# paulffm/Continuous-Time-Diffusion-Models-for-Discrete-Data

Measured on AMD Instinct MI355X. Metric: tau-leaping sample-steps/s, higher is better.
Workload: dtype bf16; 1 GPU; MNIST tauLDR U-Net TauL step (config_tauUnet_mnist: D=784, S=256, 1000-step grid); batch_per_gpu=256, global_batch=256, D=784, S=256, parallelism=sample-sharded x1, no collective in the loop

## Files before the change

continuous-time-diffusion-models-for-discrete-data_amd/csrc/row_tile.hpp:

```cpp
#pragma once
#include <type_traits>

#include "common.hpp"

namespace ctdd {

using bf16x8 = __attribute__((ext_vector_type(8))) __bf16;
using bf16x2v = __attribute__((ext_vector_type(2))) __bf16;
using f32x2v = __attribute__((ext_vector_type(2))) float;
using f32x4 = __attribute__((ext_vector_type(4))) float;
using u32x4 = __attribute__((ext_vector_type(4))) unsigned;

constexpr int RT_UNIT = 9 * 512;

__device__ inline unsigned rt_pack2(float a, float b) {
  f32x2v v = {a, b};
  return __builtin_bit_cast(unsigned, __builtin_convertvector(v, bf16x2v));
}
__device__ inline int rt_again(int v) {
  asm volatile("" : "+v"(v));
  return v;
}

__device__ __attribute__((always_inline)) inline void rt_wload9(u32x4 (&dst)[3][3], const unsigned short* __restrict__ wrow, int u) {
// ... 30 lines not shown
    for (int y = 0; y < NPT; ++y) {
      if (FULL || y < H) {
        fload(fn[y + 2], o, y + 2);
#pragma unroll
        for (int dy = 0; dy < 3; ++dy)
#pragma unroll
          for (int t = 0; t < 3; ++t)
            acc[t][y] = __builtin_amdgcn_mfma_f32_16x16x32_bf16(__builtin_bit_cast(bf16x8, slot[dy][t]), fc[y + dy], acc[t][y], 0, 0, 0);
        __builtin_amdgcn_sched_barrier(0);
      }
    }
    if (!GUARD || u + 2 < nunits) rt_wload9(slot, wrow, u + 2);
    __builtin_amdgcn_sched_barrier(0);
  };
  bf16x8 F[2][NPT + 2];
  {
    const int o = xaddr();
#pragma unroll
    for (int r = 0; r < NPT + 2; ++r)
      if (FULL || r < H + 2) fload(F[0][r], o, r);
  }
  __builtin_amdgcn_s_waitcnt(0x0F70);
  int u0 = 0;
  for (; u0 + 4 <= nunits; u0 += 2) {
    step(wr[0], F[0], F[1], u0, std::false_type{});
    step(wr[1], F[1], F[0], u0 + 1, std::false_type{});
  }
  for (; u0 < nunits; u0 += 2) {
    step(wr[0], F[0], F[1], u0, std::true_type{});
    step(wr[1], F[1], F[0], u0 + 1, std::true_type{});
  }
}

}
```

continuous-time-diffusion-models-for-discrete-data_amd/csrc/unet_rows_kernels.hip:

```cpp
#include "row_tile.hpp"
#include "../../include/ctdd_unet.h"

namespace ctdd {
namespace {

constexpr int CR_THREADS = 256, CR_N = 96, CR_BAND = 14, CR_PITCH = 32, CR_RS = 224, CR_MAXW = 28, CR_MAXC = 384, CR_PIECE = 96;
constexpr int CR_SLAB = ((CR_BAND + 2) * CR_PITCH + 2) * CR_RS;
constexpr int CR_SCALE = CR_SLAB;
constexpr int CR_RED = CR_SCALE + 2 * CR_MAXC * 4;
constexpr int CR_TOTAL = CR_RED + 2 * CR_N * 2 * 8;
constexpr int CR_FB = 12;
static_assert(CR_BAND * CR_MAXW * CR_RS <= CR_SLAB, "the output image reuses the slab");

__device__ __attribute__((always_inline)) inline void cr_fill(unsigned char* sm, const unsigned short* __restrict__ src, int cs, int pc, int coff,
                                                             int y0, int H, int W) {
  const int t = threadIdx.x, noct = pc >> 3, npl = CR_THREADS / noct;
  if (t >= noct * npl) return;
  const int oct = t % noct, pl = t / noct;
  const float* scale = (const float*)(sm + CR_SCALE) + coff + oct * 8;
  const float* shift = scale + CR_MAXC;
  const float4 sc0 = *(const float4*)scale, sc1 = *(const float4*)(scale + 4);
  const float4 sh0 = *(const float4*)shift, sh1 = *(const float4*)(shift + 4);
  const f32x2v scv[4] = {{sc0.x, sc0.y}, {sc0.z, sc0.w}, {sc1.x, sc1.y}, {sc1.z, sc1.w}};
  const f32x2v shv[4] = {{sh0.x, sh0.y}, {sh0.z, sh0.w}, {sh1.x, sh1.y}, {sh1.z, sh1.w}};
  const int rlo = y0 == 0 ? 1 : 0, rhi = H - y0 < CR_BAND + 1 ? H - y0 : CR_BAND + 1;
  const unsigned npix = (unsigned)((rhi - rlo + 1) * W), uW = (unsigned)W;
  const unsigned short* sp = src + (size_t)((y0 - 1 + rlo) * W) * cs + oct * 8;
  unsigned char* dst = sm + (1 + rlo * CR_PITCH + 1) * CR_RS + oct * 16;
  for (unsigned p0 = (unsigned)pl; p0 < npix; p0 += (unsigned)(CR_FB * npl)) {
    u32x4 u[CR_FB];
#pragma unroll
    for (int k = 0; k < CR_FB; ++k) {
      const unsigned p = p0 + (unsigned)(k * npl);
      u[k] = *(const u32x4*)(sp + (size_t)(p < npix ? p : npix - 1) * cs);
    }
#pragma unroll
    for (int k = 0; k < CR_FB; ++k) {
      const unsigned p = p0 + (unsigned)(k * npl);
      unsigned ow[4];
#pragma unroll
      for (int j = 0; j < 4; ++j) {
        const f32x2v x = {__uint_as_float(u[k][j] << 16), __uint_as_float(u[k][j] & 0xFFFF0000u)};
        f32x2v y = __builtin_elementwise_fma(x, scv[j], shv[j]);
        const f32x2v z = y * (f32x2v){-1.4426950408889634f, -1.4426950408889634f};
        const f32x2v d = (f32x2v){__builtin_amdgcn_exp2f(z.x), __builtin_amdgcn_exp2f(z.y)} + (f32x2v){1.0f, 1.0f};
        y = y * (f32x2v){__builtin_amdgcn_rcpf(d.x), __builtin_amdgcn_rcpf(d.y)};
        ow[j] = rt_pack2(y.x, y.y);
      }
      const unsigned rr = p / uW, x = p - rr * uW;
      if (p < npix) *(uint4*)(dst + (rr * CR_PITCH + x) * CR_RS) = make_uint4(ow[0], ow[1], ow[2], ow[3]);
    }
  }
}

__device__ __attribute__((always_inline)) inline void cr_gemm_skip(f32x4 (&acc)[3][CR_BAND], u32x4 (&ws)[2][3], const unsigned short* __restrict__ wrow, int nsk,
                                                                  const unsigned short* __restrict__ r1, const unsigned short* __restrict__ r2,
                                                                  int C1, int C2, int xc, int lq, int y0, int H, int W) {
  const int nc1 = C1 >> 5;
  auto gload = [&](bf16x8 (&g)[CR_BAND], int u) {
    const int ue = u < nsk ? u : nsk - 1;
    const bool two = ue >= nc1;
    const unsigned char* base = (const unsigned char*)(two ? r2 : r1);
    const int cs = two ? C2 : C1, cb = (ue - (two ? nc1 : 0)) * 32 + lq * 8;
#pragma unroll
    for (int y = 0; y < CR_BAND; ++y) {
      const int ye = y0 + y < H ? y0 + y : H - 1;
      g[y] = *(const bf16x8*)(base + (unsigned)(((ye * W + xc) * cs + cb) * 2));
    }
  };
  auto step = [&](u32x4 (&slot)[3], bf16x8 (&gc)[CR_BAND], bf16x8 (&gn)[CR_BAND], int u, auto guard) {
    constexpr bool GUARD = decltype(guard)::value;
    if (GUARD && u >= nsk) return;
    gload(gn, u + 1);
#pragma unroll
    for (int y = 0; y < CR_BAND; ++y)
#pragma unroll
      for (int t = 0; t < 3; ++t)
        acc[t][y] = __builtin_amdgcn_mfma_f32_16x16x32_bf16(__builtin_bit_cast(bf16x8, slot[t]), gc[y], acc[t][y], 0, 0, 0);
    if (!GUARD || u + 2 < nsk) rt_wload3(slot, wrow, u + 2);
    __builtin_amdgcn_sched_barrier(0);
  };
  bf16x8 G[2][CR_BAND];
  gload(G[0], 0);
  __builtin_amdgcn_s_waitcnt(0x0F70);
  int u0 = 0;
  for (; u0 + 4 <= nsk; u0 += 2) {
    step(ws[0], G[0], G[1], u0, std::false_type{});
    step(ws[1], G[1], G[0], u0 + 1, std::false_type{});
  }
  for (; u0 < nsk; u0 += 2) {
    step(ws[0], G[0], G[1], u0, std::true_type{});
    step(ws[1], G[1], G[0], u0 + 1, std::true_type{});
  }
}

#ifdef CTDD_ROWS_STAMPS
#define CR_STAMP(i_)                                                                                      \
  do {                                                                                                    \
    unsigned long long t_;                                                                                \
    asm volatile("s_memtime %0\n\ts_waitcnt lgkmcnt(0)" : "=s"(t_)::"memory");                            \
    if (threadIdx.x == 0) ((unsigned long long*)a.out_stats)[(size_t)blockIdx.x * 8 + (i_)] = t_;         \
  } while (0)
#else
#define CR_STAMP(i_)
#endif

template <bool SKIP>
__global__ __launch_bounds__(CR_THREADS, 1) void k_conv_rows(const ctdd_conv_rows_args a) {
  extern __shared__ __attribute__((aligned(16))) unsigned char sm[];
  const int t = threadIdx.x;
  const int H = a.H, W = a.W, HW = H * W, C1 = a.C1, C2 = a.C2, C = C1 + C2;
  const int nbands = (H + CR_BAND - 1) / CR_BAND;
  const int b = blockIdx.x / nbands, y0 = (blockIdx.x - b * nbands) * CR_BAND;
  const int lane = t & 63, wv = t >> 6, lj = lane & 15, lq = lane >> 4, cg = wv >> 1, hh = wv & 1;
  const int nu3 = 3 * (C >> 5), nsk = SKIP ? (a.RC1 + a.RC2) >> 5 : 0;
  const unsigned short* wrow = (const unsigned short*)a.w + (size_t)cg * ((size_t)nu3 * RT_UNIT + (size_t)nsk * 1536) + lane * 8;
  u32x4 wr[2][3][3];
  CR_STAMP(0);

  rt_wload9(wr[0], wrow, 0);
  rt_wload9(wr[1], wrow, 1);
  for (int v = t; v < (CR_SLAB >> 4); v += CR_THREADS) *(uint4*)(sm + v * 16) = make_uint4(0, 0, 0, 0);
  {
    float* scale = (float*)(sm + CR_SCALE);
    float* shift = scale + CR_MAXC;
    const int cgp = C / a.G;
    for (int c = t; c < C; c += CR_THREADS) {
      const int g0 = (c / cgp) * cgp;
      double s = 0.0, q = 0.0;
      for (int j = g0; j < g0 + cgp; ++j) {
        const double* st = j < C1 ? a.st1 + ((size_t)b * C1 + j) * 2 : a.st2 + ((size_t)b * C2 + (j - C1)) * 2;
        s += st[0]; q += st[1];
      }
      const double n = (double)cgp * (double)HW;
      const double mean = s / n;
      const double var = fmax(q / n - mean * mean, 0.0);
      const float rstd = (float)(1.0 / sqrt(var + (double)a.eps));
      scale[c] = rstd * a.gamma[c];
      shift[c] = a.beta[c] - (float)mean * rstd * a.gamma[c];
    }
  }
  __syncthreads();
  CR_STAMP(1);

  const int fb = (1 + 16 * hh + lj) * CR_RS + lq * 16;
  f32x4 acc[3][CR_BAND];
#pragma unroll
  for (int tt = 0; tt < 3; ++tt)
#pragma unroll
    for (int y = 0; y < CR_BAND; ++y) acc[tt][y] = (f32x4){0.0f, 0.0f, 0.0f, 0.0f};

  int ub = 0;
  for (int s = 0; s < (C2 ? 2 : 1); ++s) {
    const int cs = s ? C2 : C1, coff = s ? C1 : 0;
    const unsigned short* src = (const unsigned short*)(s ? a.s2_bf16 : a.s1_bf16) + (size_t)b * HW * cs;
    for (int c0 = 0; c0 < cs; c0 += CR_PIECE) {
      const int pc = cs - c0 < CR_PIECE ? cs - c0 : CR_PIECE, nun = 3 * (pc >> 5);
      cr_fill(sm, src + c0, cs, pc, coff + c0, y0, H, W);
      __syncthreads();
      rt_gemm_rows<true, CR_RS, CR_PITCH>(acc, wr, wrow + (size_t)ub * RT_UNIT, nun, sm, fb, CR_BAND);
      __syncthreads();
      ub += nun;
      if (ub < nu3) {
        rt_wload9(wr[0], wrow + (size_t)ub * RT_UNIT, 0);
        rt_wload9(wr[1], wrow + (size_t)ub * RT_UNIT, 1);
      }
    }
  }
  CR_STAMP(2);

  if constexpr (SKIP) {
    const unsigned short* wsk = wrow + (size_t)nu3 * RT_UNIT;
    u32x4 ws[2][3];
    rt_wload3(ws[0], wsk, 0);
    if (nsk > 1) rt_wload3(ws[1], wsk, 1);
    const int cs_ = 16 * hh + rt_again(lj), xc = cs_ < 1 ? 0 : (cs_ > W ? W - 1 : cs_ - 1);
    cr_gemm_skip(acc, ws, wsk, nsk, (const unsigned short*)a.r1_bf16 + (size_t)b * HW * a.RC1,
                 (const unsigned short*)a.r2_bf16 + (size_t)b * HW * a.RC2, a.RC1, a.RC2, xc, lq, y0, H, W);
  }
  CR_STAMP(3);

  const int col = 16 * hh + rt_again(lj);
  const bool own = col >= 1 && col <= W;
  const int x2 = own ? col - 1 : 0;
  const int nrows = H - y0 < CR_BAND ? H - y0 : CR_BAND;
  double* red = (double*)(sm + CR_RED);
  uint2 rr[3][CR_BAND] = {};
  const bool res = !SKIP && a.res_bf16;
  if (res) {
    const unsigned short* rp = (const unsigned short*)a.res_bf16 + (size_t)b * HW * CR_N + cg * 48 + lq * 4;
#pragma unroll
    for (int y = 0; y < CR_BAND; ++y) {
      const unsigned short* rpy = rp + (size_t)(((y < nrows ? y0 + y : H - 1)) * W + x2) * CR_N;
#pragma unroll
      for (int tt = 0; tt < 3; ++tt) rr[tt][y] = *(const uint2*)(rpy + tt * 16);
    }
  }
#pragma unroll
  for (int tt = 0; tt < 3; ++tt) {
    const int n = cg * 48 + tt * 16 + lq * 4;
    const float4 bv = *(const float4*)(a.bias + n);
    const float4 tb = a.tbias ? *(const float4*)(a.tbias + (size_t)b * a.tb_stride + n) : make_float4(0.0f, 0.0f, 0.0f, 0.0f);
    const float add[4] = {bv.x + tb.x, bv.y + tb.y, bv.z + tb.z, bv.w + tb.w};
    const uint2 (&r)[CR_BAND] = rr[tt];
    float s[4] = {0.0f, 0.0f, 0.0f, 0.0f}, q[4] = {0.0f, 0.0f, 0.0f, 0.0f};
#pragma unroll
    for (int y = 0; y < CR_BAND; ++y) {
      if (y < nrows && own) {
        const f32x4 v = acc[tt][y];
        float o[4] = {v[0] + add[0], v[1] + add[1], v[2] + add[2], v[3] + add[3]};
        if (res) {
          o[0] += __uint_as_float(r[y].x << 16); o[1] += __uint_as_float(r[y].x & 0xFFFF0000u);
          o[2] += __uint_as_float(r[y].y << 16); o[3] += __uint_as_float(r[y].y & 0xFFFF0000u);
        }
#pragma unroll
        for (int i = 0; i < 4; ++i) { s[i] += o[i]; q[i] = fmaf(o[i], o[i], q[i]); }
        *(uint2*)(sm + (y * W + x2) * CR_RS + n * 2) = make_uint2(rt_pack2(o[0], o[1]), rt_pack2(o[2], o[3]));
      }
    }
#ifndef CTDD_ROWS_STAMPS
    if (a.out_stats) {
#pragma unroll
      for (int i = 0; i < 4; ++i) {
        double ds = (double)s[i], dq = (double)q[i];
#pragma unroll
        for (int m = 1; m < 16; m <<= 1) { ds += __shfl_xor(ds, m, WAVE); dq += __shfl_xor(dq, m, WAVE); }
        if (lj == 0) { red[(hh * CR_N + n + i) * 2] = ds; red[(hh * CR_N + n + i) * 2 + 1] = dq; }
      }
    }
#endif
  }
  __syncthreads();
  CR_STAMP(4);
  {
    constexpr int npc = CR_N / 8;
    unsigned short* out = (unsigned short*)a.out_bf16 + ((size_t)b * HW + (size_t)y0 * W) * CR_N;
    for (int v = t; v < nrows * W * npc; v += CR_THREADS) {
      const int p = v / npc, c0 = (v - p * npc) * 8;
      *(uint4*)(out + (size_t)p * CR_N + c0) = *(const uint4*)(sm + p * CR_RS + c0 * 2);
    }
#ifndef CTDD_ROWS_STAMPS
    if (a.out_stats && t < 2 * CR_N) atomicAdd(a.out_stats + (size_t)b * CR_N * 2 + t, red[t] + red[2 * CR_N + t]);
#endif
  }
  CR_STAMP(5);
}

}
}

using namespace ctdd;

extern "C" int ctdd_unet_conv_rows(const void* args_, int f32, void* stream) {
  CTDD_REQUIRE(args_, CTDD_EINVAL, "ctdd_unet_conv_rows: null arguments");
  const ctdd_conv_rows_args& a = *(const ctdd_conv_rows_args*)args_;
  CTDD_REQUIRE(f32 == 0, CTDD_ERANGE, "ctdd_unet_conv_rows: bf16 inference only (the fp32 mode keeps GroupNorm and convolution apart)");
  CTDD_REQUIRE(a.B > 0 && a.H > 0 && a.W >= 1 && a.W <= CR_MAXW, CTDD_ERANGE,
               "ctdd_unet_conv_rows: a grid of %dx%d pixels does not fit the row tiles (1 <= W <= 28)", a.H, a.W);
  const int nbands = (a.H + CR_BAND - 1) / CR_BAND;
  CTDD_REQUIRE((int64_t)a.B * nbands < ((int64_t)1 << 31) && (int64_t)a.H * a.W * CR_MAXC < ((int64_t)1 << 30), CTDD_ERANGE,
               "ctdd_unet_conv_rows: B=%d, %dx%d is over the 32-bit index range of the kernel", a.B, a.H, a.W);
  const int C = a.C1 + a.C2;
  CTDD_REQUIRE(a.N == CR_N && a.C1 > 0 && a.C1 % 32 == 0 && a.C2 >= 0 && a.C2 % 32 == 0 && C <= CR_MAXC && a.RC1 >= 0 && a.RC1 % 32 == 0 &&
                   a.RC2 >= 0 && a.RC2 % 32 == 0 && (a.RC2 == 0 || a.RC1 > 0) && a.RC1 + a.RC2 <= CR_MAXC, CTDD_ERANGE,
               "ctdd_unet_conv_rows: channel counts off the tile (N=%d, C1=%d, C2=%d, RC1=%d, RC2=%d; N = 96, sources in multiples of 32, <= 384 in all)",
               a.N, a.C1, a.C2, a.RC1, a.RC2);
  CTDD_REQUIRE(a.G > 0 && C % a.G == 0, CTDD_EINVAL, "ctdd_unet_conv_rows: %d groups do not divide %d channels", a.G, C);
  CTDD_REQUIRE(a.s1_bf16 && (a.C2 == 0 || a.s2_bf16) && (a.RC1 == 0 || a.r1_bf16) && (a.RC2 == 0 || a.r2_bf16) && a.gamma && a.beta && a.w &&
                   a.bias && a.out_bf16, CTDD_EINVAL, "ctdd_unet_conv_rows: null pointer");
  CTDD_REQUIRE(a.st1 && (a.C2 == 0 || a.st2), CTDD_EINVAL, "ctdd_unet_conv_rows: a GroupNorm source without statistics");
  auto al16 = [](const void* p) { return ((uintptr_t)p & 15) == 0; };
  CTDD_REQUIRE(al16(a.s1_bf16) && al16(a.s2_bf16) && al16(a.r1_bf16) && al16(a.r2_bf16) && al16(a.res_bf16) && al16(a.w) && al16(a.out_bf16) &&
                   al16(a.bias) && al16(a.tbias) && a.tb_stride % 4 == 0, CTDD_EINVAL, "ctdd_unet_conv_rows: tensors must be 16-byte aligned");
  CTDD_REQUIRE(!(a.RC1 > 0 && a.res_bf16), CTDD_EINVAL, "ctdd_unet_conv_rows: 1x1 segments and a residual in one call");
  static bool attr_done[2][16] = {};
  if (a.RC1 > 0) {
    ensure_lds_ceiling((const void*)k_conv_rows<true>, attr_done[1]);
    hipLaunchKernelGGL(k_conv_rows<true>, dim3(a.B * nbands), dim3(CR_THREADS), (size_t)CR_TOTAL, (hipStream_t)stream, a);
  } else {
    ensure_lds_ceiling((const void*)k_conv_rows<false>, attr_done[0]);
    hipLaunchKernelGGL(k_conv_rows<false>, dim3(a.B * nbands), dim3(CR_THREADS), (size_t)CR_TOTAL, (hipStream_t)stream, a);
  }
  return finish_launch("k_conv_rows");
}
```

continuous-time-diffusion-models-for-discrete-data_amd/ctdd/native.py:

```python
import ctypes as C
import os

import torch

_HERE = os.path.dirname(os.path.dirname(os.path.abspath(__file__)))
_LIB = None

BRANCH_CTELBO, BRANCH_CRM = 0, 1
LOGIT_TYPES = {"direct": 0, "reverse_prob": 1, "reverse_logscale": 2}
STEP_ORDINAL, STEP_CORRECTOR, STEP_COUNT_RAW, STEP_CRM, STEP_COUNT_JUMPS, STEP_BF16, STEP_LOGITS_BF16 = 1, 2, 4, 8, 16, 32, 64


class CtddError(RuntimeError):
    pass


def lib_path():
    return os.environ.get("CTDD_LIBRARY") or os.path.join(_HERE, "libctdd.so")


_P, _I, _F, _U64, _U32, _I64 = C.c_void_p, C.c_int, C.c_float, C.c_uint64, C.c_uint32, C.c_int64
_SIGS = {
    "ctdd_abi_version": ([], _I),
    "ctdd_last_error": ([], C.c_char_p),
# ... 25 lines not shown
    "ctdd_s256_step_table_bytes": ([], _I64),
    "ctdd_s256_prepare": ([_P, _P, _F, _I, _P, _P, _P, _P], _I),
    "ctdd_s256_prepare_crm": ([_P, _P, _I, _P, _P, _P, _P], _I),
    "ctdd_tauleap_step_s256": ([_P, _P, _P, _P, _P, _P, _F, _F, _U32, _U64, _U64, _I, _I, _P, _P, _P, _P], _I),
    "ctdd_tauleap_step_s256_rows": ([_P, _P, _P, _P, _P, _P, _F, _F, _U32, _U64, _U64, _I, _I, _P, _I, _P, _P, _P, _P], _I),
    "ctdd_crm_loss": ([_P, _P, _P, _P, _I, _I, _I, _I, _F, _F, _P, _P, _P, _P], _I),
    "ctdd_ctelbo_scratch_bytes": ([_I, _I, _I], _I64),
    "ctdd_ctelbo_loss": ([_P, _P, _P, _P, _P, _P, _I, _I, _I, _F, _F, _F, _P, _P, _P, _P], _I),
    "ctdd_ctelbo_loss_terms": ([_P, _P, _P, _P, _P, _P, _I, _I, _I, _F, _F, _F, _F, _P, _P, _P, _P], _I),
    "ctdd_ctelbo_loss_window": ([_P, _P, _P, _P, _P, _P, _I, _I, _I, _I, _I, _F, _F, _F, _F, _P, _P, _P, _P], _I),
    "ctdd_ctelbo_loss_masked": ([_P, _P, _P, _P, _P, _P, _P, _I, _I, _I, _F, _F, _F, _F, _P, _P, _P, _P], _I),
    "ctdd_score_elbo_loss": ([_P, _P, _P, _P, _P, _P, _I, _I, _I, _F, _F, _P, _P, _P, _P], _I),
    "ctdd_crm_loss_ll": ([_P, _P, _P, _I, _I, _I, _I, _F, _P, _P, _P, _P], _I),
    "ctdd_score_elbo_loss_ll": ([_P, _P, _P, _P, _P, _P, _I, _I, _I, _F, _F, _P, _P, _P, _P], _I),
    "ctdd_logprob_bwd": ([_I, _P, _P, _P, _P, _P, _F, _I, _I, _I, _P, _P, _P, _P], _I),
    "ctdd_crm_loss_masked": ([_P, _P, _P, _P, _P, _I, _I, _I, _I, _F, _F, _P, _P, _P, _P], _I),
    "ctdd_crm_loss_ll_masked": ([_P, _P, _P, _P, _I, _I, _I, _I, _F, _P, _P, _P, _P], _I),
    "ctdd_score_elbo_loss_masked": ([_P, _P, _P, _P, _P, _P, _P, _I, _I, _I, _F, _F, _P, _P, _P, _P], _I),
    "ctdd_score_elbo_loss_ll_masked": ([_P, _P, _P, _P, _P, _P, _P, _I, _I, _I, _F, _F, _P, _P, _P, _P], _I),
    "ctdd_opt_chunk_elems": ([], _I),
    "ctdd_adam_ema_step": ([_P, _P, _I, _F, _F, _F, _F, _I64, _F, _F, _P, _P], _I),
    "ctdd_grad_sumsq": ([_P, _P, _I, _P, _I, _P], _I),
    "ctdd_adam_ema_apply": ([_P, _P, _I, _F, _F, _F, _F, _I64, _F, _F, _P, _P], _I),
    "ctdd_d3pm_scratch_bytes": ([_I, _I, _I], _I64),
    "ctdd_d3pm_loss": ([_P, _P, _P, _P, _P, _P, _P, _I, _I, _I, _F, _F, _F, _P, _P, _P, _P, _P, _P], _I),
    "ctdd_d3pm_step": ([_P, _P, _P, _P, _P, _I, _I, _I, _I, _F, _P, _U64, _U64, _P, _P, _P, _P], _I),
    "ctdd_absorb_noise": ([_P, _P, _I, _I, _I, _U64, _U64, _P, _P], _I),
    "ctdd_absorb_scratch_bytes": ([], _I64),
    "ctdd_absorb_elbo_loss": ([_P, _P, _P, _P, _F, _I, _I, _I, _I, _P, _P, _P, _P], _I),
    "ctdd_absorb_step": ([_P, _P, _I, _I, _I, _I, _F, _U32, _U64, _U64, _P, _P, _P], _I),
}
UNET_EXPORTS = ("ctdd_unet_conv", "ctdd_unet_conv_patch", "ctdd_unet_conv_res", "ctdd_unet_conv_ring", "ctdd_unet_conv_up_phases", "ctdd_unet_upsample2x", "ctdd_unet_first_conv", "ctdd_unet_gn_apply", "ctdd_unet_gn_onepass", "ctdd_unet_channel_stats",
                "ctdd_unet_time", "ctdd_unet_time_uniform", "ctdd_unet_attention", "ctdd_unet_logistic_head", "ctdd_unet_resblock_small",
                "ctdd_unet_resblock_mid", "ctdd_unet_conv_rows", "ctdd_unet_conv_rows_head", "ctdd_unet_attention_block")
HOLLOW_EXPORTS = ("ctdd_gemm_bf16", "ctdd_hollow_small_linear", "ctdd_hollow_embed", "ctdd_hollow_layernorm", "ctdd_hollow_add", "ctdd_hollow_put_rows", "ctdd_hollow_attention", "ctdd_hollow_attention_bf16")
UNET_TRAIN_EXPORTS = ("ctdd_unet_wgrad", "ctdd_unet_gn_bwd", "ctdd_unet_dropout", "ctdd_unet_colsum", "ctdd_unet_sum_batch", "ctdd_unet_sum_jobs", "ctdd_unet_accumulate",
                      "ctdd_unet_downsum2x", "ctdd_unet_upsample2x_f32", "ctdd_unet_cast_rows", "ctdd_unet_attention_bwd",
                      "ctdd_unet_first_conv_wgrad", "ctdd_unet_first_conv_wgrad_scratch", "ctdd_unet_pack_weights",
                      "ctdd_unet_unpack_grads")
HOLLOW_TRAIN_EXPORTS = ("ctdd_hollow_layernorm_bwd", "ctdd_hollow_attention_train", "ctdd_hollow_attention_bwd", "ctdd_hollow_attention_train_bf16", "ctdd_hollow_attention_bwd_bf16", "ctdd_hollow_act", "ctdd_hollow_relu_bf16", "ctdd_hollow_colsum", "ctdd_hollow_dropout",
                        "ctdd_hollow_embed_bwd")
BERT_EXPORTS = ("ctdd_bert_embed", "ctdd_bert_gather", "ctdd_bert_attention_short",
                "ctdd_bert_embed_bwd", "ctdd_bert_gather_bwd",
                "ctdd_bert_embed_enum_bwd", "ctdd_bert_gather_enum_bwd",
                "ctdd_bert_attention_short_train", "ctdd_bert_attention_short_bwd")
EXPORTS = tuple(_SIGS) + UNET_EXPORTS + HOLLOW_EXPORTS + UNET_TRAIN_EXPORTS + HOLLOW_TRAIN_EXPORTS + BERT_EXPORTS


def load():
    global _LIB
    if _LIB is None:
        path = lib_path()
        if not os.path.exists(path):
            raise CtddError(f"{path} not found: build it with `python __graft_entry__.py` "
                            "(hipcc --offload-arch=gfx950); there is no CPU fallback")
        lib = C.CDLL(path)
        for name, (argt, rest) in _SIGS.items():
            fn = getattr(lib, name)
            fn.argtypes, fn.restype = argt, rest
        _LIB = lib
    return _LIB


def _ptr(t, dtype=None, name="tensor"):
    if t is None:
        return None
    if not isinstance(t, torch.Tensor):
# ... 639 lines not shown
```

continuous-time-diffusion-models-for-discrete-data_amd/ctdd/unet_engine.py:

```python
import contextlib
import ctypes as C

import torch

from . import native
from .plan_launch import bound_launch, graph_capture, ptr

_P, _I, _F = C.c_void_p, C.c_int, C.c_float
SEG_3x3, SEG_1x1, SEG_3x3_S2, SEG_3x3_UP = 0, 1, 2, 3


class _Seg(C.Structure):
    _fields_ = [("hi", _P), ("f32", _P), ("C", _I), ("kind", _I)]


class _ConvArgs(C.Structure):
    _fields_ = [("seg", _Seg * 3), ("nseg", _I), ("w_hi", _P), ("w_f32", _P), ("B", _I), ("H", _I), ("W", _I),
                ("Hin", _I), ("Win", _I), ("N", _I), ("Ktot", _I), ("bias", _P), ("tbias", _P), ("tb_stride", _I),
                ("res_f32", _P), ("res_bf16", _P), ("out_f32", _P), ("out_hi", _P), ("stats", _P), ("logits_C", _I),
                ("ksplit", _I), ("acc_buf", _P), ("act", _I), ("out_lo", _P)]


class _FirstArgs(C.Structure):
    _fields_ = [("x64", _P), ("x32", _P), ("lo", _F), ("hi", _F), ("w", _P), ("bias", _P), ("B", _I), ("Cin", _I),
# ... 19 lines not shown


class _TimeArgs(C.Structure):
    _fields_ = [("t", _P), ("B", _I), ("ch", _I), ("tdim", _I), ("w1", _P), ("b1", _P), ("w2", _P), ("b2", _P),
                ("hid", _P), ("act", _P)]


class _AttnArgs(C.Structure):
    _fields_ = [("qkv", _P), ("B", _I), ("T", _I), ("C", _I), ("heads", _I), ("out_hi", _P), ("out_f32", _P)]


class _AttnBlockArgs(C.Structure):
    _fields_ = [("an_bf16", _P), ("x_bf16", _P), ("w_qkv", _P), ("b_qkv", _P), ("w_proj", _P), ("b_proj", _P), ("B", _I), ("T", _I),
                ("C", _I), ("heads", _I), ("out_bf16", _P)]


class _LogisticArgs(C.Structure):
    _fields_ = [("net", _P), ("x0", _P), ("B", _I), ("C", _I), ("HW", _I), ("S", _I), ("fix", _I), ("out", _P), ("fast", _I), ("out_bf16", _P)]


_sigs_done = False


def _lib():
    global _sigs_done
    lib = native.load()
    if not _sigs_done:
        for name, argt in (("ctdd_unet_conv", [_P, _I, _I, _I, _P]), ("ctdd_unet_conv_patch", [_P, _I, _I, _I, _P]), ("ctdd_unet_conv_res", [_P, _I, _P]), ("ctdd_unet_conv_ring", [_P, _I, _P]),
                           ("ctdd_unet_conv_up_phases", [_P, _I, _P]), ("ctdd_unet_upsample2x", [_P, _I, _I, _I, _I, _P, _P]), ("ctdd_unet_first_conv", [_P, _P]),
                           ("ctdd_unet_gn_apply", [_P, _P]), ("ctdd_unet_gn_onepass", [_P, _I, _I, _P]), ("ctdd_unet_channel_stats", [_P, _I, _I, _I, _P, _P]),
                           ("ctdd_unet_time", [_P, _P, _P, _I, _P, _P]), ("ctdd_unet_time_uniform", [_P, _P, _P, _I, _P, _P]),
                           ("ctdd_unet_attention", [_P, _P]), ("ctdd_unet_attention_block", [_P, _I, _P]),
                           ("ctdd_unet_resblock_small", [_P, _I, _P]),
                           ("ctdd_unet_resblock_mid", [_P, _I, _P]), ("ctdd_unet_conv_rows", [_P, _I, _P]),
                           ("ctdd_unet_conv_rows_head", [_P, _I, _P]),
                           ("ctdd_unet_logistic_head", [_P, _P])):
            fn = getattr(lib, name)
            fn.argtypes, fn.restype = argt, _I
        _sigs_done = True
    return lib


def _unwrap(net):
    return net.module if hasattr(net, "module") and net.__class__.__name__ == "DistributedDataParallel" else net


def supports(model):
    net = _unwrap(getattr(model, "net", None))
    return (net is not None and net.__class__.__name__ == "UNet" and not model.padding
            and model.cfg.model.model_output in ("logits", "logistic_pars"))


def training_supported(model):
    if getattr(model.cfg.model, "engine_train", "hip") != "hip" or not supports(model):
        return False
    net = _unwrap(model.net)
    return net.channel % 16 == 0 and all((net.channel * int(m_)) % 16 == 0 for m_ in model.cfg.model.ch_mult)



def resblock_small_covers(H, W, cs, cout, G1, G2):
    Ct = sum(cs)
    if H * W > 64 or W > 8 or cout != 192 or len(cs) > 2 or any(c % 64 for c in cs) or Ct > 384 or Ct % G1 or cout % G2:
        return False
    if H * W > 16 and (H - 1) * (W + 2) + W > 80:
        return False
    rs_a, rs_2, prows = Ct * 2 + 32, cout * 2 + 32, (H + 2) * (W + 2)
# ... 302 lines not shown
            self.launch(lib.ctdd_unet_gn_onepass, C.byref(a), 0, self.gn_threads, label=f"gn1 {srcs[0].H}x{srcs[0].W} C={Ct} ({len(srcs)} src)")
        else:
            self.launch(lib.ctdd_unet_gn_apply, C.byref(a), label=f"gn {srcs[0].H}x{srcs[0].W} C={Ct} ({len(srcs)} src)")
        if tc is not None:
            tc.record_gn(self, srcs, norm, swish, eps, HW, out, drop_p)
        return out

    def conv_rows(self, srcs, norm, segs, wsrc, bias, out, tb=None, res=None, raws=()):
        eng, lib, B = self.eng, self.lib, self.B
        Hc, Wc, N = srcs[0].H, srcs[0].W, out.C
        cs, rcs = [s_.C for s_ in srcs], [s_.C for s_ in raws]
        a = _ConvRowsArgs()
        for i, s_ in enumerate(srcs):
            setattr(a, f"s{i + 1}_bf16", ptr(s_.hi))
            setattr(a, f"C{i + 1}", s_.C)
            self.stats_views.append((a, s_.stats, f"st{i + 1}"))
        for i, s_ in enumerate(raws):
            setattr(a, f"r{i + 1}_bf16", ptr(s_.hi))
            setattr(a, f"RC{i + 1}", s_.C)
        g, b_ = norm.weight.detach().float().contiguous(), norm.bias.detach().float().contiguous()
        a.gamma, a.beta, a.G, a.eps = ptr(g), ptr(b_), norm.num_groups, norm.eps
        w, _ = eng._pack(pack_conv_rows_weights(eng._w2d(wsrc, segs), cs, rcs))
        a.w, a.bias = ptr(w), ptr(bias)
        if tb is not None:
            a.tbias, a.tb_stride = tb
        if res is not None:
            a.res_bf16 = ptr(res.hi)
        a.out_bf16 = ptr(out.hi)
        if out.stats is not None and not out.stats_by_gn:
            self.stats_views.append((a, out.stats, "out_stats"))
        a.B, a.H, a.W, a.N = B, Hc, Wc, N
        self.keep.extend([g, b_, w, bias, a])
        Ktot = w.shape[1]
        self.launch(lib.ctdd_unet_conv_rows, C.byref(a), 0, label=f"{Hc}x{Wc} K={Ktot} N={N} gn+conv rows C={cs} raw={rcs}",
                    flops=2 * B * Hc * Wc * N * Ktot)

    def conv_rows_head(self, src, norm, oc, logits):
        eng, B = self.eng, self.B
        N, C1 = oc.weight.shape[0], src.C
        a = _ConvRowsArgs()
        a.s1_bf16, a.C1 = ptr(src.hi), C1
        self.stats_views.append((a, src.stats, "st1"))
        g, b_ = norm.weight.detach().float().contiguous(), norm.bias.detach().float().contiguous()
        a.gamma, a.beta, a.G, a.eps = ptr(g), ptr(b_), norm.num_groups, norm.eps
        w, _ = eng._pack(pack_conv_rows_head_weights(eng._w2d([(oc.weight, 0)], [(None, C1, SEG_3x3)]), C1))
        bias = oc.bias.detach().float().contiguous()
        a.w, a.bias, a.out_bf16 = ptr(w), ptr(bias), ptr(logits)
        a.B, a.H, a.W, a.N = B, src.H, src.W, N
        self.keep.extend([g, b_, w, bias, a])
        self.launch(self.lib.ctdd_unet_conv_rows_head, C.byref(a), 0, label=f"{src.H}x{src.W} K={9 * C1} N={N} gn+conv rows head C={[C1]}",
                    flops=2 * B * src.H * src.W * N * 9 * C1)

    def conv2_operands(self, rb, a2, srcs):
        tc = self.tc
        segs, wsrc, bias_params = [(a2, rb.conv2.weight.shape[0], SEG_3x3)], [(rb.conv2.weight, 0)], [rb.conv2.bias]
        bias = rb.conv2.bias.detach().float()
        if rb.skip is not None:
            c_ = 0
            for s_ in srcs:
                segs.append((s_, s_.C, SEG_1x1))
                wsrc.append((rb.skip.weight, c_))
                c_ += s_.C
            bias_params.append(rb.skip.bias)
            bias = tc.summed_bias(bias_params) if tc is not None else bias + rb.skip.bias.detach().float()
        return segs, wsrc, bias_params, bias.contiguous()

    def resblock_fused(self, rb, srcs, mid=False):
# ... 580 lines not shown
```

include/ctdd_unet.h:

```cpp
#ifndef CTDD_UNET_H
#define CTDD_UNET_H
#include <stdint.h>
#ifdef __cplusplus
extern "C" {
#endif

#define CTDD_SEG_3x3 0
#define CTDD_SEG_1x1 1
#define CTDD_SEG_3x3_S2 2
#define CTDD_SEG_3x3_UP 3
#define CTDD_SEG_3x3_S2T 4

typedef struct { const void* hi; const float* f32; int C, kind; } ctdd_conv_seg;
typedef struct {
  ctdd_conv_seg seg[3]; int nseg;
  const void* w_hi; const float* w_f32;
  int B, H, W, Hin, Win, N, Ktot;
  const float* bias; const float* tbias; int tb_stride;
  const float* res_f32; const void* res_bf16;
  float* out_f32; void* out_hi; double* stats; int logits_C;
  int ksplit; float* acc_buf;
  int act;
  void* out_lo;
} ctdd_conv_args;
// ... 11 lines not shown
int ctdd_unet_first_conv(const void* first_conv_args, void* stream);

typedef struct {
  const float* s1_f32; const void* s1_bf16; const double* st1; int C1;
  const float* s2_f32; const void* s2_bf16; const double* st2; int C2;
  const float* gamma; const float* beta; int B, HW, G; float eps; int swish; void* out_hi; float* out_f32;
} ctdd_gn_args;
int ctdd_unet_gn_apply(const void* gn_args, void* stream);
int ctdd_unet_gn_onepass(const void* gn_args, int slab_channels, int max_threads, void* stream);
int ctdd_unet_channel_stats(const float* x, int B, int HW, int C, double* stats, void* stream);

typedef struct {
  const void* s1_bf16; const void* s2_bf16; int C1, C2;
  const float* gamma1; const float* beta1; const float* gamma2; const float* beta2; int G1, G2; float eps1, eps2;
  const void* w1; const float* bias1; const float* tbias; int tb_stride;
  const void* w2; const float* bias2;
  int skip;
  int B, H, W, N; void* out_bf16;
} ctdd_resblock_args;
int ctdd_unet_resblock_small(const void* resblock_args, int f32, void* stream);
int ctdd_unet_resblock_mid(const void* resblock_args, int f32, void* stream);

typedef struct {
  const void* s1_bf16; const double* st1; int C1;
  const void* s2_bf16; const double* st2; int C2;
  const float* gamma; const float* beta; int G; float eps;
  const void* w; const float* bias; const float* tbias; int tb_stride;
  const void* r1_bf16; int RC1; const void* r2_bf16; int RC2;
  const void* res_bf16;
  void* out_bf16; double* out_stats;
  int B, H, W, N;
} ctdd_conv_rows_args;
int ctdd_unet_conv_rows(const void* conv_rows_args, int f32, void* stream);
int ctdd_unet_conv_rows_head(const void* conv_rows_args, int f32, void* stream);

typedef struct {
  const float* t; int B, ch, tdim;
  const float* w1; const float* b1; const float* w2; const float* b2;
  float* hid; float* act;
} ctdd_time_args;
int ctdd_unet_time(const void* time_args, const float* proj_w, const float* proj_b, int Ntot, float* proj_out, void* stream);
int ctdd_unet_time_uniform(const void* time_args, const float* proj_w, const float* proj_b, int Ntot, float* proj_out, void* stream);

typedef struct { const float* qkv; int B, T, C, heads; void* out_hi; float* out_f32; } ctdd_attn_args;
int ctdd_unet_attention(const void* attn_args, void* stream);

typedef struct {
  const void* an_bf16; const void* x_bf16;
  const void* w_qkv; const float* b_qkv;
  const void* w_proj; const float* b_proj;
  int B, T, C, heads; void* out_bf16;
} ctdd_attn_block_args;
int ctdd_unet_attention_block(const void* attn_block_args, int f32, void* stream);

typedef struct { const float* net; const float* x0; int B, C, HW, S, fix; float* out;
                 int fast;
                 void* out_bf16;    } ctdd_logistic_args;
int ctdd_unet_logistic_head(const void* logistic_args, void* stream);

#ifdef __cplusplus
}
#endif
#endif
```

Before: 134,200 sample-steps/s.

## Split conv-rows band across 8 waves with single-buffered row fragments

The fused GroupNorm+conv rows kernel now runs 8 waves per block by default, with each half of the waves owning half of the 14-row band (7 rows each). This halves the accumulators per wave, and a new single-buffer GEMM variant reuses the fragment registers in place of double buffering them. Together these are meant to cut register pressure and add latency hiding inside the single resident block. The upper waves hand their partial GroupNorm statistics to the lower waves through leftover slab space in LDS, at the cost of an extra barrier. The 4-wave path is kept behind a config switch.

Result: faster. 140,000 sample-steps/s, median of 6 (+4.3%).

```diff
diff --git a/continuous-time-diffusion-models-for-discrete-data_amd/csrc/row_tile.hpp b/continuous-time-diffusion-models-for-discrete-data_amd/csrc/row_tile.hpp
--- a/continuous-time-diffusion-models-for-discrete-data_amd/csrc/row_tile.hpp
+++ b/continuous-time-diffusion-models-for-discrete-data_amd/csrc/row_tile.hpp
@@ -86,4 +86,56 @@
   }
 }
 
+template <int RS, int PITCH, int NPT>
+__device__ __attribute__((always_inline)) inline void rt_gemm_rows_1buf(f32x4 (&acc)[3][NPT], u32x4 (&wr)[2][3][3], const unsigned short* __restrict__ wrow,
+                                                                       int nunits, const unsigned char* sm, int fb) {
+  int un = 0, dxn = 0, cbn = 0;
+  auto xaddr = [&]() {
+    const int o = fb + (dxn - 1) * RS + cbn * 64;
+    const bool more = un + 1 < nunits, wrap = dxn == 2;
+    un += more ? 1 : 0;
+    cbn += more && wrap ? 1 : 0;
+    dxn = more ? (wrap ? 0 : dxn + 1) : dxn;
+    return o;
+  };
+  auto fload = [&](bf16x8& f, int o, int r) { f = *(const bf16x8*)(sm + o + r * (PITCH * RS)); };
+  bf16x8 F[NPT + 2];
+  auto step = [&](u32x4 (&slot)[3][3], int u, auto guard) {
+    constexpr bool GUARD = decltype(guard)::value;
+    if (GUARD && u >= nunits) return;
+    const int o = xaddr();
+#pragma unroll
+    for (int y = 0; y < NPT; ++y) {
+#pragma unroll
+      for (int dy = 0; dy < 3; ++dy)
+#pragma unroll
+        for (int t = 0; t < 3; ++t)
+          acc[t][y] = __builtin_amdgcn_mfma_f32_16x16x32_bf16(__builtin_bit_cast(bf16x8, slot[dy][t]), F[y + dy], acc[t][y], 0, 0, 0);
+      fload(F[y], o, y);
+      if (y == NPT - 1) {
+        fload(F[NPT], o, NPT);
+        fload(F[NPT + 1], o, NPT + 1);
+      }
+      __builtin_amdgcn_sched_barrier(0);
+    }
+    if (!GUARD || u + 2 < nunits) rt_wload9(slot, wrow, u + 2);
+    __builtin_amdgcn_sched_barrier(0);
+  };
+  {
+    const int o = xaddr();
+#pragma unroll
+    for (int r = 0; r < NPT + 2; ++r) fload(F[r], o, r);
+  }
+  __builtin_amdgcn_s_waitcnt(0x0F70);
+  int u0 = 0;
+  for (; u0 + 4 <= nunits; u0 += 2) {
+    step(wr[0], u0, std::false_type{});
+    step(wr[1], u0 + 1, std::false_type{});
+  }
+  for (; u0 < nunits; u0 += 2) {
+    step(wr[0], u0, std::true_type{});
+    step(wr[1], u0 + 1, std::true_type{});
+  }
 }
+
+}
diff --git a/continuous-time-diffusion-models-for-discrete-data_amd/csrc/unet_rows_kernels.hip b/continuous-time-diffusion-models-for-discrete-data_amd/csrc/unet_rows_kernels.hip
--- a/continuous-time-diffusion-models-for-discrete-data_amd/csrc/unet_rows_kernels.hip
+++ b/continuous-time-diffusion-models-for-discrete-data_amd/csrc/unet_rows_kernels.hip
@@ -4,17 +4,19 @@
 namespace ctdd {
 namespace {
 
-constexpr int CR_THREADS = 256, CR_N = 96, CR_BAND = 14, CR_PITCH = 32, CR_RS = 224, CR_MAXW = 28, CR_MAXC = 384, CR_PIECE = 96;
+constexpr int CR_N = 96, CR_BAND = 14, CR_PITCH = 32, CR_RS = 224, CR_MAXW = 28, CR_MAXC = 384, CR_PIECE = 96;
 constexpr int CR_SLAB = ((CR_BAND + 2) * CR_PITCH + 2) * CR_RS;
 constexpr int CR_SCALE = CR_SLAB;
 constexpr int CR_RED = CR_SCALE + 2 * CR_MAXC * 4;
 constexpr int CR_TOTAL = CR_RED + 2 * CR_N * 2 * 8;
 constexpr int CR_FB = 12;
-static_assert(CR_BAND * CR_MAXW * CR_RS <= CR_SLAB, "the output image reuses the slab");
-
+constexpr int CR_CARRY = CR_BAND * CR_MAXW * CR_RS;
+static_assert(CR_CARRY + 4 * 3 * 2 * 64 * 16 <= CR_SLAB, "the output image and the upper waves' partial sums reuse the slab");
+
+template <int THREADS, int FB>
 __device__ __attribute__((always_inline)) inline void cr_fill(unsigned char* sm, const unsigned short* __restrict__ src, int cs, int pc, int coff,
                                                              int y0, int H, int W) {
-  const int t = threadIdx.x, noct = pc >> 3, npl = CR_THREADS / noct;
+  const int t = threadIdx.x, noct = pc >> 3, npl = THREADS / noct;
   if (t >= noct * npl) return;
   const int oct = t % noct, pl = t / noct;
   const float* scale = (const float*)(sm + CR_SCALE) + coff + oct * 8;
@@ -27,15 +29,15 @@
   const unsigned npix = (unsigned)((rhi - rlo + 1) * W), uW = (unsigned)W;
   const unsigned short* sp = src + (size_t)((y0 - 1 + rlo) * W) * cs + oct * 8;
   unsigned char* dst = sm + (1 + rlo * CR_PITCH + 1) * CR_RS + oct * 16;
-  for (unsigned p0 = (unsigned)pl; p0 < npix; p0 += (unsigned)(CR_FB * npl)) {
-    u32x4 u[CR_FB];
-#pragma unroll
-    for (int k = 0; k < CR_FB; ++k) {
+  for (unsigned p0 = (unsigned)pl; p0 < npix; p0 += (unsigned)(FB * npl)) {
+    u32x4 u[FB];
+#pragma unroll
+    for (int k = 0; k < FB; ++k) {
       const unsigned p = p0 + (unsigned)(k * npl);
       u[k] = *(const u32x4*)(sp + (size_t)(p < npix ? p : npix - 1) * cs);
     }
 #pragma unroll
-    for (int k = 0; k < CR_FB; ++k) {
+    for (int k = 0; k < FB; ++k) {
       const unsigned p = p0 + (unsigned)(k * npl);
       unsigned ow[4];
 #pragma unroll
@@ -53,34 +55,35 @@
   }
 }
 
-__device__ __attribute__((always_inline)) inline void cr_gemm_skip(f32x4 (&acc)[3][CR_BAND], u32x4 (&ws)[2][3], const unsigned short* __restrict__ wrow, int nsk,
+template <int NPT>
+__device__ __attribute__((always_inline)) inline void cr_gemm_skip(f32x4 (&acc)[3][NPT], u32x4 (&ws)[2][3], const unsigned short* __restrict__ wrow, int nsk,
                                                                   const unsigned short* __restrict__ r1, const unsigned short* __restrict__ r2,
                                                                   int C1, int C2, int xc, int lq, int y0, int H, int W) {
   const int nc1 = C1 >> 5;
-  auto gload = [&](bf16x8 (&g)[CR_BAND], int u) {
+  auto gload = [&](bf16x8 (&g)[NPT], int u) {
     const int ue = u < nsk ? u : nsk - 1;
     const bool two = ue >= nc1;
     const unsigned char* base = (const unsigned char*)(two ? r2 : r1);
     const int cs = two ? C2 : C1, cb = (ue - (two ? nc1 : 0)) * 32 + lq * 8;
 #pragma unroll
-    for (int y = 0; y < CR_BAND; ++y) {
+    for (int y = 0; y < NPT; ++y) {
       const int ye = y0 + y < H ? y0 + y : H - 1;
       g[y] = *(const bf16x8*)(base + (unsigned)(((ye * W + xc) * cs + cb) * 2));
     }
   };
-  auto step = [&](u32x4 (&slot)[3], bf16x8 (&gc)[CR_BAND], bf16x8 (&gn)[CR_BAND], int u, auto guard) {
+  auto step = [&](u32x4 (&slot)[3], bf16x8 (&gc)[NPT], bf16x8 (&gn)[NPT], int u, auto guard) {
     constexpr bool GUARD = decltype(guard)::value;
     if (GUARD && u >= nsk) return;
     gload(gn, u + 1);
 #pragma unroll
-    for (int y = 0; y < CR_BAND; ++y)
+    for (int y = 0; y < NPT; ++y)
 #pragma unroll
       for (int t = 0; t < 3; ++t)
         acc[t][y] = __builtin_amdgcn_mfma_f32_16x16x32_bf16(__builtin_bit_cast(bf16x8, slot[t]), gc[y], acc[t][y], 0, 0, 0);
     if (!GUARD || u + 2 < nsk) rt_wload3(slot, wrow, u + 2);
     __builtin_amdgcn_sched_barrier(0);
   };
-  bf16x8 G[2][CR_BAND];
+  bf16x8 G[2][NPT];
   gload(G[0], 0);
   __builtin_amdgcn_s_waitcnt(0x0F70);
   int u0 = 0;
@@ -105,14 +108,17 @@
 #define CR_STAMP(i_)
 #endif
 
-template <bool SKIP>
-__global__ __launch_bounds__(CR_THREADS, 1) void k_conv_rows(const ctdd_conv_rows_args a) {
+template <bool SKIP, int WAVES>
+__global__ __launch_bounds__(WAVES * 64, 1) void k_conv_rows(const ctdd_conv_rows_args a) {
+  static_assert(WAVES == 4 || WAVES == 8, "one or two row halves");
+  constexpr int CR_THREADS = WAVES * 64, NPT = CR_BAND * 4 / WAVES;
   extern __shared__ __attribute__((aligned(16))) unsigned char sm[];
   const int t = threadIdx.x;
   const int H = a.H, W = a.W, HW = H * W, C1 = a.C1, C2 = a.C2, C = C1 + C2;
   const int nbands = (H + CR_BAND - 1) / CR_BAND;
   const int b = blockIdx.x / nbands, y0 = (blockIdx.x - b * nbands) * CR_BAND;
-  const int lane = t & 63, wv = t >> 6, lj = lane & 15, lq = lane >> 4, cg = wv >> 1, hh = wv & 1;
+  const int lane = t & 63, wv = t >> 6, lj = lane & 15, lq = lane >> 4, cg = WAVES == 8 ? (wv >> 1) & 1 : wv >> 1, hh = wv & 1;
+  const int rh = WAVES == 8 ? __builtin_amdgcn_readfirstlane(wv >> 2) : 0, yw = y0 + NPT * rh;
   const int nu3 = 3 * (C >> 5), nsk = SKIP ? (a.RC1 + a.RC2) >> 5 : 0;
   const unsigned short* wrow = (const unsigned short*)a.w + (size_t)cg * ((size_t)nu3 * RT_UNIT + (size_t)nsk * 1536) + lane * 8;
   u32x4 wr[2][3][3];
@@ -143,12 +149,12 @@
   __syncthreads();
   CR_STAMP(1);
 
-  const int fb = (1 + 16 * hh + lj) * CR_RS + lq * 16;
-  f32x4 acc[3][CR_BAND];
+  const int fb = (1 + 16 * hh + lj) * CR_RS + lq * 16 + rh * (NPT * CR_PITCH * CR_RS);
+  f32x4 acc[3][NPT];
 #pragma unroll
   for (int tt = 0; tt < 3; ++tt)
 #pragma unroll
-    for (int y = 0; y < CR_BAND; ++y) acc[tt][y] = (f32x4){0.0f, 0.0f, 0.0f, 0.0f};
+    for (int y = 0; y < NPT; ++y) acc[tt][y] = (f32x4){0.0f, 0.0f, 0.0f, 0.0f};
 
   int ub = 0;
   for (int s = 0; s < (C2 ? 2 : 1); ++s) {
@@ -156,9 +162,12 @@
     const unsigned short* src = (const unsigned short*)(s ? a.s2_bf16 : a.s1_bf16) + (size_t)b * HW * cs;
     for (int c0 = 0; c0 < cs; c0 += CR_PIECE) {
       const int pc = cs - c0 < CR_PIECE ? cs - c0 : CR_PIECE, nun = 3 * (pc >> 5);
-      cr_fill(sm, src + c0, cs, pc, coff + c0, y0, H, W);
+      cr_fill<CR_THREADS, CR_FB * 4 / WAVES>(sm, src + c0, cs, pc, coff + c0, y0, H, W);
       __syncthreads();
-      rt_gemm_rows<true, CR_RS, CR_PITCH>(acc, wr, wrow + (size_t)ub * RT_UNIT, nun, sm, fb, CR_BAND);
+      if constexpr (WAVES == 8)
+        rt_gemm_rows_1buf<CR_RS, CR_PITCH>(acc, wr, wrow + (size_t)ub * RT_UNIT, nun, sm, fb);
+      else
+        rt_gemm_rows<true, CR_RS, CR_PITCH>(acc, wr, wrow + (size_t)ub * RT_UNIT, nun, sm, fb, NPT);
       __syncthreads();
       ub += nun;
       if (ub < nu3) {
@@ -176,7 +185,7 @@
     if (nsk > 1) rt_wload3(ws[1], wsk, 1);
     const int cs_ = 16 * hh + rt_again(lj), xc = cs_ < 1 ? 0 : (cs_ > W ? W - 1 : cs_ - 1);
     cr_gemm_skip(acc, ws, wsk, nsk, (const unsigned short*)a.r1_bf16 + (size_t)b * HW * a.RC1,
-                 (const unsigned short*)a.r2_bf16 + (size_t)b * HW * a.RC2, a.RC1, a.RC2, xc, lq, y0, H, W);
+                 (const unsigned short*)a.r2_bf16 + (size_t)b * HW * a.RC2, a.RC1, a.RC2, xc, lq, yw, H, W);
   }
   CR_STAMP(3);
 
@@ -184,14 +193,16 @@
   const bool own = col >= 1 && col <= W;
   const int x2 = own ? col - 1 : 0;
   const int nrows = H - y0 < CR_BAND ? H - y0 : CR_BAND;
+  const int nr = WAVES == 8 ? (nrows - NPT * rh < 0 ? 0 : (nrows - NPT * rh < NPT ? nrows - NPT * rh : NPT)) : nrows;
   double* red = (double*)(sm + CR_RED);
-  uint2 rr[3][CR_BAND] = {};
+  float4* carry = (float4*)(sm + CR_CARRY) + (wv & 3) * (3 * 2 * 64) + lane;
+  uint2 rr[3][NPT] = {};
   const bool res = !SKIP && a.res_bf16;
   if (res) {
     const unsigned short* rp = (const unsigned short*)a.res_bf16 + (size_t)b * HW * CR_N + cg * 48 + lq * 4;
 #pragma unroll
-    for (int y = 0; y < CR_BAND; ++y) {
-      const unsigned short* rpy = rp + (size_t)(((y < nrows ? y0 + y : H - 1)) * W + x2) * CR_N;
+    for (int y = 0; y < NPT; ++y) {
+      const unsigned short* rpy = rp + (size_t)(((y < nr ? yw + y : H - 1)) * W + x2) * CR_N;
 #pragma unroll
       for (int tt = 0; tt < 3; ++tt) rr[tt][y] = *(const uint2*)(rpy + tt * 16);
     }
@@ -202,24 +213,59 @@
     const float4 bv = *(const float4*)(a.bias + n);
     const float4 tb = a.tbias ? *(const float4*)(a.tbias + (size_t)b * a.tb_stride + n) : make_float4(0.0f, 0.0f, 0.0f, 0.0f);
     const float add[4] = {bv.x + tb.x, bv.y + tb.y, bv.z + tb.z, bv.w + tb.w};
-    const uint2 (&r)[CR_BAND] = rr[tt];
+    const uint2 (&r)[NPT] = rr[tt];
     float s[4] = {0.0f, 0.0f, 0.0f, 0.0f}, q[4] = {0.0f, 0.0f, 0.0f, 0.0f};
 #pragma unroll
-    for (int y = 0; y < CR_BAND; ++y) {
-      if (y < nrows && own) {
+    for (int y = 0; y < NPT; ++y) {
+      if (y < nr && own) {
         const f32x4 v = acc[tt][y];
         float o[4] = {v[0] + add[0], v[1] + add[1], v[2] + add[2], v[3] + add[3]};
         if (res) {
           o[0] += __uint_as_float(r[y].x << 16); o[1] += __uint_as_float(r[y].x & 0xFFFF0000u);
           o[2] += __uint_as_float(r[y].y << 16); o[3] += __uint_as_float(r[y].y & 0xFFFF0000u);
         }
-#pragma unroll
-        for (int i = 0; i < 4; ++i) { s[i] += o[i]; q[i] = fmaf(o[i], o[i], q[i]); }
-        *(uint2*)(sm + (y * W + x2) * CR_RS + n * 2) = make_uint2(rt_pack2(o[0], o[1]), rt_pack2(o[2], o[3]));
+        if (WAVES == 8 && rh) {
+          acc[tt][y] = (f32x4){o[0], o[1], o[2], o[3]};
+        } else {
+#pragma unroll
+          for (int i = 0; i < 4; ++i) { s[i] += o[i]; q[i] = fmaf(o[i], o[i], q[i]); }
+        }
+        *(uint2*)(sm + ((NPT * rh + y) * W + x2) * CR_RS + n * 2) = make_uint2(rt_pack2(o[0], o[1]), rt_pack2(o[2], o[3]));
       }
     }
 #ifndef CTDD_ROWS_STAMPS
     if (a.out_stats) {
+      if constexpr (WAVES == 4) {
+#pragma unroll
+        for (int i = 0; i < 4; ++i) {
+          double ds = (double)s[i], dq = (double)q[i];
+#pragma unroll
+          for (int m = 1; m < 16; m <<= 1) { ds += __shfl_xor(ds, m, WAVE); dq += __shfl_xor(dq, m, WAVE); }
+          if (lj == 0) { red[(hh * CR_N + n + i) * 2] = ds; red[(hh * CR_N + n + i) * 2 + 1] = dq; }
+        }
+      } else if (!rh) {
+        carry[(tt * 2) * 64] = make_float4(s[0], s[1], s[2], s[3]);
+        carry[(tt * 2 + 1) * 64] = make_float4(q[0], q[1], q[2], q[3]);
+      }
+    }
+#endif
+  }
+  __syncthreads();
+  CR_STAMP(4);
+#ifndef CTDD_ROWS_STAMPS
+  if (WAVES == 8 && rh && a.out_stats) {
+#pragma unroll
+    for (int tt = 0; tt < 3; ++tt) {
+      const float4 cs_ = carry[(tt * 2) * 64], cq = carry[(tt * 2 + 1) * 64];
+      float s[4] = {cs_.x, cs_.y, cs_.z, cs_.w}, q[4] = {cq.x, cq.y, cq.z, cq.w};
+#pragma unroll
+      for (int y = 0; y < NPT; ++y) {
+        if (y < nr && own) {
+#pragma unroll
+          for (int i = 0; i < 4; ++i) { s[i] += acc[tt][y][i]; q[i] = fmaf(acc[tt][y][i], acc[tt][y][i], q[i]); }
+        }
+      }
+      const int n = cg * 48 + tt * 16 + lq * 4;
 #pragma unroll
       for (int i = 0; i < 4; ++i) {
         double ds = (double)s[i], dq = (double)q[i];
@@ -228,10 +274,8 @@
         if (lj == 0) { red[(hh * CR_N + n + i) * 2] = ds; red[(hh * CR_N + n + i) * 2 + 1] = dq; }
       }
     }
+  }
 #endif
-  }
-  __syncthreads();
-  CR_STAMP(4);
   {
     constexpr int npc = CR_N / 8;
     unsigned short* out = (unsigned short*)a.out_bf16 + ((size_t)b * HW + (size_t)y0 * W) * CR_N;
@@ -240,6 +284,7 @@
       *(uint4*)(out + (size_t)p * CR_N + c0) = *(const uint4*)(sm + p * CR_RS + c0 * 2);
     }
 #ifndef CTDD_ROWS_STAMPS
+    if (WAVES == 8) __syncthreads();
     if (a.out_stats && t < 2 * CR_N) atomicAdd(a.out_stats + (size_t)b * CR_N * 2 + t, red[t] + red[2 * CR_N + t]);
 #endif
   }
@@ -251,7 +296,8 @@
 
 using namespace ctdd;
 
-extern "C" int ctdd_unet_conv_rows(const void* args_, int f32, void* stream) {
+template <int WAVES>
+static int launch_conv_rows(const void* args_, int f32, void* stream) {
   CTDD_REQUIRE(args_, CTDD_EINVAL, "ctdd_unet_conv_rows: null arguments");
   const ctdd_conv_rows_args& a = *(const ctdd_conv_rows_args*)args_;
   CTDD_REQUIRE(f32 == 0, CTDD_ERANGE, "ctdd_unet_conv_rows: bf16 inference only (the fp32 mode keeps GroupNorm and convolution apart)");
@@ -275,11 +321,14 @@
   CTDD_REQUIRE(!(a.RC1 > 0 && a.res_bf16), CTDD_EINVAL, "ctdd_unet_conv_rows: 1x1 segments and a residual in one call");
   static bool attr_done[2][16] = {};
   if (a.RC1 > 0) {
-    ensure_lds_ceiling((const void*)k_conv_rows<true>, attr_done[1]);
-    hipLaunchKernelGGL(k_conv_rows<true>, dim3(a.B * nbands), dim3(CR_THREADS), (size_t)CR_TOTAL, (hipStream_t)stream, a);
+    ensure_lds_ceiling((const void*)k_conv_rows<true, WAVES>, attr_done[1]);
+    hipLaunchKernelGGL((k_conv_rows<true, WAVES>), dim3(a.B * nbands), dim3(WAVES * 64), (size_t)CR_TOTAL, (hipStream_t)stream, a);
   } else {
-    ensure_lds_ceiling((const void*)k_conv_rows<false>, attr_done[0]);
-    hipLaunchKernelGGL(k_conv_rows<false>, dim3(a.B * nbands), dim3(CR_THREADS), (size_t)CR_TOTAL, (hipStream_t)stream, a);
+    ensure_lds_ceiling((const void*)k_conv_rows<false, WAVES>, attr_done[0]);
+    hipLaunchKernelGGL((k_conv_rows<false, WAVES>), dim3(a.B * nbands), dim3(WAVES * 64), (size_t)CR_TOTAL, (hipStream_t)stream, a);
   }
   return finish_launch("k_conv_rows");
 }
+
+extern "C" int ctdd_unet_conv_rows(const void* args_, int f32, void* stream) { return launch_conv_rows<8>(args_, f32, stream); }
+extern "C" int ctdd_unet_conv_rows_w4(const void* args_, int f32, void* stream) { return launch_conv_rows<4>(args_, f32, stream); }
diff --git a/continuous-time-diffusion-models-for-discrete-data_amd/ctdd/native.py b/continuous-time-diffusion-models-for-discrete-data_amd/ctdd/native.py
--- a/continuous-time-diffusion-models-for-discrete-data_amd/ctdd/native.py
+++ b/continuous-time-diffusion-models-for-discrete-data_amd/ctdd/native.py
@@ -81,7 +81,7 @@
 }
 UNET_EXPORTS = ("ctdd_unet_conv", "ctdd_unet_conv_patch", "ctdd_unet_conv_res", "ctdd_unet_conv_ring", "ctdd_unet_conv_up_phases", "ctdd_unet_upsample2x", "ctdd_unet_first_conv", "ctdd_unet_gn_apply", "ctdd_unet_gn_onepass", "ctdd_unet_channel_stats",
                 "ctdd_unet_time", "ctdd_unet_time_uniform", "ctdd_unet_attention", "ctdd_unet_logistic_head", "ctdd_unet_resblock_small",
-                "ctdd_unet_resblock_mid", "ctdd_unet_conv_rows", "ctdd_unet_conv_rows_head", "ctdd_unet_attention_block")
+                "ctdd_unet_resblock_mid", "ctdd_unet_conv_rows", "ctdd_unet_conv_rows_w4", "ctdd_unet_conv_rows_head", "ctdd_unet_attention_block")
 HOLLOW_EXPORTS = ("ctdd_gemm_bf16", "ctdd_hollow_small_linear", "ctdd_hollow_embed", "ctdd_hollow_layernorm", "ctdd_hollow_add", "ctdd_hollow_put_rows", "ctdd_hollow_attention", "ctdd_hollow_attention_bf16")
 UNET_TRAIN_EXPORTS = ("ctdd_unet_wgrad", "ctdd_unet_gn_bwd", "ctdd_unet_dropout", "ctdd_unet_colsum", "ctdd_unet_sum_batch", "ctdd_unet_sum_jobs", "ctdd_unet_accumulate",
                       "ctdd_unet_downsum2x", "ctdd_unet_upsample2x_f32", "ctdd_unet_cast_rows", "ctdd_unet_attention_bwd",
diff --git a/continuous-time-diffusion-models-for-discrete-data_amd/ctdd/unet_engine.py b/continuous-time-diffusion-models-for-discrete-data_amd/ctdd/unet_engine.py
--- a/continuous-time-diffusion-models-for-discrete-data_amd/ctdd/unet_engine.py
+++ b/continuous-time-diffusion-models-for-discrete-data_amd/ctdd/unet_engine.py
@@ -75,7 +75,7 @@
                            ("ctdd_unet_time", [_P, _P, _P, _I, _P, _P]), ("ctdd_unet_time_uniform", [_P, _P, _P, _I, _P, _P]),
                            ("ctdd_unet_attention", [_P, _P]), ("ctdd_unet_attention_block", [_P, _I, _P]),
                            ("ctdd_unet_resblock_small", [_P, _I, _P]),
-                           ("ctdd_unet_resblock_mid", [_P, _I, _P]), ("ctdd_unet_conv_rows", [_P, _I, _P]),
+                           ("ctdd_unet_resblock_mid", [_P, _I, _P]), ("ctdd_unet_conv_rows", [_P, _I, _P]), ("ctdd_unet_conv_rows_w4", [_P, _I, _P]),
                            ("ctdd_unet_conv_rows_head", [_P, _I, _P]),
                            ("ctdd_unet_logistic_head", [_P, _P])):
             fn = getattr(lib, name)
@@ -444,7 +444,10 @@
         a.B, a.H, a.W, a.N = B, Hc, Wc, N
         self.keep.extend([g, b_, w, bias, a])
         Ktot = w.shape[1]
-        self.launch(lib.ctdd_unet_conv_rows, C.byref(a), 0, label=f"{Hc}x{Wc} K={Ktot} N={N} gn+conv rows C={cs} raw={rcs}",
+        waves = int(getattr(eng.cfg.model, "conv_rows_waves", 8))
+        if waves not in (4, 8):
+            raise ValueError(f"cfg.model.conv_rows_waves = {waves}: 4 or 8")
+        self.launch(lib.ctdd_unet_conv_rows if waves == 8 else lib.ctdd_unet_conv_rows_w4, C.byref(a), 0, label=f"{Hc}x{Wc} K={Ktot} N={N} gn+conv rows C={cs} raw={rcs}",
                     flops=2 * B * Hc * Wc * N * Ktot)
 
     def conv_rows_head(self, src, norm, oc, logits):
diff --git a/include/ctdd_unet.h b/include/ctdd_unet.h
--- a/include/ctdd_unet.h
+++ b/include/ctdd_unet.h
@@ -67,6 +67,7 @@
   int B, H, W, N;
 } ctdd_conv_rows_args;
 int ctdd_unet_conv_rows(const void* conv_rows_args, int f32, void* stream);
+int ctdd_unet_conv_rows_w4(const void* conv_rows_args, int f32, void* stream);
 int ctdd_unet_conv_rows_head(const void* conv_rows_args, int f32, void* stream);
 
 typedef struct {
```
